# impromptuRong/hd_yolo

Hardware: AMD Instinct MI355X
Metric: tiles/sec (640x640) fwd+bwd (higher is better)
Workload: dtype bf16; 1 GPU; metayolo yolov5s 8-class nuclei, 640x640 RGB tiles, batch 64/GPU, train step = fwd + DetLoss + bwd + all-reduce + SGD(nesterov); global_batch=64, parallelism=dp1, world_size=1, backend=none, hw_queues=4

## Files before the change

### hd_yolo_amd/_ext.py

```python
import os

from . import _header, _lib
from ._header import HdyError

MEASURE_HEADER = os.path.join(os.path.dirname(_header.HEADER_PATH), 'hdyolo_measure.h')
_M = _header.read(MEASURE_HEADER)
SIGNATURES = _M.functions
PARAMS = _M.params
CONSTANTS = _M.constants
MEASURE_REVISION, MEASURE_COLS, MEASURE_MAX_SIDE = (CONSTANTS['HDY_MEASURE_' + n] for n in ('REVISION', 'COLS', 'MAX_SIDE'))

_bound = None


def load():
    global _bound
    lib = _lib.load()
    if _bound is not lib:
        rebuild = 'rebuild with `python -m hd_yolo_amd.build --force`'
        for name, (res, args) in SIGNATURES.items():
            fn = getattr(lib, name, None)
            if fn is None:
                raise HdyError(f'{_lib.LIB_PATH} does not export {name} (include/hdyolo_measure.h): it was built before the extension header '
                               f'existed; {rebuild}')
            fn.restype, fn.argtypes = res, args
        got = lib.hdy_measure_revision()
        if got != MEASURE_REVISION:
            raise HdyError(f'{_lib.LIB_PATH} was built for revision {got} of include/hdyolo_measure.h, this binding is written for '
                           f'{MEASURE_REVISION} (HDY_MEASURE_REVISION): {rebuild}')
        _bound = lib
    return lib


def call(name, *args):
    lib = load()
    rc = getattr(lib, name)(*args)
    if rc != 0:
        raise HdyError(f'{name} failed (status {rc}): {lib.hdy_last_error().decode()}')
```

### hd_yolo_amd/build.py

```python
import os
import subprocess
import sys
from concurrent.futures import ThreadPoolExecutor

HERE = os.path.dirname(os.path.abspath(__file__))
CSRC = os.path.join(HERE, 'csrc')
OUT = os.path.join(CSRC, 'build')
LIB = os.path.join(OUT, 'libhdyolo_hip.so')
SOURCES = ['api.hip', 'conv_dispatch.hip', 'conv_igemm.hip', 'conv3x3.hip', 'conv3x3_c128.hip', 'conv3x3s2.hip', 'conv_deep.hip', 'conv_stem.hip', 'conv_wgrad.hip', 'conv_wgrad3x3.hip', 'conv_wgrad_deep.hip', 'conv_dgrad_s2.hip', 'conv1x1_bwd.hip', 'bn_act.hip', 'pool.hip', 'detect.hip', 'nms_grid.hip', 'slide.hip', 'augment.hip', 'augment_masks.hip', 'score.hip', 'paste.hip', 'mask_score.hip', 'measure.hip', 'loss.hip', 'roi.hip', 'seg.hip', 'optim.hip', 'exec.hip']
FLAGS = ['--offload-arch=gfx950', '-O3', '-fPIC', '-std=c++17', '-ffp-contract=off', '-Wall', '-Wno-unused-function',
         '-I' + CSRC, '-I' + os.path.join(os.path.dirname(HERE), 'include')]


def _newer(a, bs):
    return os.path.exists(a) and all(os.path.getmtime(a) >= os.path.getmtime(b) for b in bs)


def build(force=False, verbose=True):
    os.makedirs(OUT, exist_ok=True)
    headers = [os.path.join(CSRC, h) for h in os.listdir(CSRC) if h.endswith('.h')]
    headers += [os.path.join(os.path.dirname(HERE), 'include', h) for h in ('hdyolo.h', 'hdyolo_measure.h')]
    hipcc = os.environ.get('HIPCC', '/opt/rocm/bin/hipcc')

    def compile_one(src):
        s = os.path.join(CSRC, src)
        o = os.path.join(OUT, src.replace('.hip', '.o'))
        if not force and _newer(o, [s] + headers):
            return o
        cmd = [hipcc] + FLAGS + ['-c', s, '-o', o]
        if verbose:
            print(' '.join(cmd), flush=True)
        subprocess.check_call(cmd)
        return o

    with ThreadPoolExecutor(max_workers=min(6, os.cpu_count() or 1)) as ex:
        objs = list(ex.map(compile_one, SOURCES))
    if force or not _newer(LIB, objs):
        cmd = [hipcc, '--offload-arch=gfx950', '-shared', '-fPIC', '-o', LIB] + objs
        if verbose:
            print(' '.join(cmd), flush=True)
        subprocess.check_call(cmd)
    return LIB


if __name__ == '__main__':
    print(build(force='--force' in sys.argv))
```

### hd_yolo_amd/csrc/api.hip

```cpp
#include <stdarg.h>
#include <stdio.h>
#include <stdlib.h>
#include <string.h>

#include <atomic>

#include "common.h"
#include "hdyolo_internal.h"
#include "hdyolo.h"

int hdy_pack_weight_launch(const hdy_pack_desc& d, hipStream_t st);
int hdy_pack_batch_launch(const hdy_pack_desc* table, int n, int total_blocks, hipStream_t st);

static thread_local char g_err[512] = "";

void hdy_set_error(const char* fmt, ...) {
    va_list ap;
    va_start(ap, fmt);
    vsnprintf(g_err, sizeof(g_err), fmt, ap);
    va_end(ap);
}

namespace {
struct OptDef { const char* name; int def; bool flag; };
const OptDef g_opt_def[HDY_OPT_COUNT] = {
    {"HDY_NO_CLASS_WALK", 0, true}, {"HDY_NO_CONV3X3", 0, true}, {"HDY_C3_GRID", 0, false}, {"HDY_NO_CONV3X3S2", 0, false},
    {"HDY_NO_DGRAD_S2", 0, false}, {"HDY_TILE_INTERLEAVE", 1, false}, {"HDY_NO_BIG_TILES", 0, true}, {"HDY_NO_STEM_KERNEL", 0, true},
    {"HDY_WGRAD_BLOCKS", 512, false}, {"HDY_NO_STEM_WGRAD", 0, true}, {"HDY_NO_WGRAD3X3", 0, true}, 
    {"HDY_LOSS_GRID", 2048, false}, {"HDY_NO_DEEP", 0, true}, {"HDY_NO_WGRAD_DEEP", 0, true}, {"HDY_DEEP_BN", 0, false}, {"HDY_DEEP_DEBUG", 0, false}, {"HDY_DEEP_ALL", 1, false}, {"HDY_DEEP_MIN_TILES", 160, false}, {"HDY_DEEP_WALK", 2, false}, {"HDY_NO_BN_REDUCE4", 0, true},
    {"HDY_WGRAD_TILE", 0, false}, {"HDY_SPPF_NO_KEYS", 0, true}, {"HDY_WGRAD_DEEP_KMIN", 192, false}, {"HDY_NO_CONV3X3_C128", 0, true}, {"HDY_NO_F1X1_96", 0, true},
    {"HDY_AP_CHUNK", 0, false}, {"HDY_AP_NO_PRUNE", 0, true},
};
std::atomic<int> g_opt[HDY_OPT_COUNT];
std::once_flag g_opt_once;
void opt_init() {
    std::call_once(g_opt_once, [] {
        for (int i = 0; i < HDY_OPT_COUNT; ++i) {
            const char* v = getenv(g_opt_def[i].name);
            g_opt[i].store(v ? (g_opt_def[i].flag ? 1 : atoi(v)) : g_opt_def[i].def, std::memory_order_relaxed);
        }
    });
}
int opt_index(const char* name) {
    for (int i = 0; name && i < HDY_OPT_COUNT; ++i)
        if (!strcmp(name, g_opt_def[i].name)) return i;
    return -1;
}
thread_local char g_disp_last[64] = "";
std::mutex g_disp_mu;
char g_disp_log[32768] = "";
size_t g_disp_len = 0;
thread_local char g_disp_copy[32768] = "";
}

int hdy_opt(int id) {
    opt_init();
    return g_opt[id].load(std::memory_order_relaxed);
}

void hdy_note_dispatch(const char* what) {
    snprintf(g_disp_last, sizeof(g_disp_last), "%s", what);
    const size_t n = strlen(g_disp_last);
    std::lock_guard<std::mutex> lock(g_disp_mu);
    if (g_disp_len + n + 2 < sizeof(g_disp_log)) {
// ... 148 lines not shown
```

### hd_yolo_amd/csrc/common.h

```cpp
#pragma once
#include <hip/hip_runtime.h>
#include <stdint.h>
#include <stddef.h>

#include <mutex>

#define HDY_OK 0
#define HDY_EINVAL (-1)
#define HDY_EUNSUPPORTED (-2)

enum { HDY_F32 = 0, HDY_BF16 = 1 };

void hdy_set_error(const char* fmt, ...);

enum HdyOption {
    HDY_OPT_NO_CLASS_WALK,
    HDY_OPT_NO_CONV3X3,
    HDY_OPT_C3_GRID,
    HDY_OPT_NO_CONV3X3S2,
    HDY_OPT_NO_DGRAD_S2,
    HDY_OPT_TILE_INTERLEAVE,
    HDY_OPT_NO_BIG_TILES,
    HDY_OPT_NO_STEM_KERNEL,
    HDY_OPT_WGRAD_BLOCKS,
    HDY_OPT_NO_STEM_WGRAD,
    HDY_OPT_NO_WGRAD3X3,
    HDY_OPT_LOSS_GRID,
    HDY_OPT_NO_DEEP,
    HDY_OPT_NO_WGRAD_DEEP,
    HDY_OPT_DEEP_BN,
    HDY_OPT_DEEP_DEBUG,
    HDY_OPT_DEEP_ALL,
    HDY_OPT_DEEP_MIN_TILES,
    HDY_OPT_DEEP_WALK,
    HDY_OPT_NO_BN_REDUCE4,
    HDY_OPT_WGRAD_TILE,
    HDY_OPT_SPPF_NO_KEYS,
    HDY_OPT_WGRAD_DEEP_KMIN,
    HDY_OPT_NO_CONV3X3_C128,
    HDY_OPT_NO_F1X1_96,
    HDY_OPT_AP_CHUNK,
    HDY_OPT_AP_NO_PRUNE,
    HDY_OPT_COUNT
};
int hdy_opt(int id);

void hdy_note_dispatch(const char* what);

#define HDY_ARG(cond, ...)                 \
    do {                                   \
        if (!(cond)) {                     \
            hdy_set_error(__VA_ARGS__);    \
            return HDY_EINVAL;             \
        }                                  \
    } while (0)

#define HDY_LAUNCH_CHECK(what)                                                       \
    do {                                                                             \
        hipError_t e__ = hipGetLastError();                                          \
        if (e__ != hipSuccess) {                                                     \
            hdy_set_error("%s: launch failed: %s", what, hipGetErrorString(e__));    \
            return (int)e__;                                                         \
        }                                                                            \
    } while (0)

typedef __bf16 bf16_t;
typedef int i32x4 __attribute__((ext_vector_type(4)));
typedef float f32x4 __attribute__((ext_vector_type(4)));
typedef __bf16 bf16x8 __attribute__((ext_vector_type(8)));
typedef __bf16 bf16x4 __attribute__((ext_vector_type(4)));

#if defined(__HIPCC__)
__device__ __forceinline__ float row_sum16(float v) {
#ifdef HDY_ROW_SUM_SHFL
    for (int m = 1; m < 16; m <<= 1) v += __shfl_xor(v, m);
// ... 131 lines not shown
```

### hd_yolo_amd/csrc/exec.hip

```cpp
#include <hip/hip_runtime.h>
#include <stdlib.h>
#include <string.h>

#include <mutex>
#include <tuple>
#include <type_traits>
#include <utility>
#include <vector>

#include "common.h"
#include "hdyolo.h"

namespace {

typedef unsigned long long u64;

#define HDY_HIP(call)                                                                  \
    do {                                                                               \
        hipError_t e__ = (call);                                                       \
        if (e__ != hipSuccess) {                                                       \
            hdy_set_error("exec: %s failed: %s", #call, hipGetErrorString(e__));       \
            return (int)e__;                                                           \
        }                                                                              \
    } while (0)

template <typename T>
T arg_from(u64 v) {
    if constexpr (std::is_pointer_v<T>) {
        return reinterpret_cast<T>((uintptr_t)v);
    } else if constexpr (std::is_same_v<T, float>) {
        const unsigned u = (unsigned)v;
        float f;
        __builtin_memcpy(&f, &u, 4);
        return f;
    } else if constexpr (std::is_same_v<T, double>) {
        double d;
        __builtin_memcpy(&d, &v, 8);
        return d;
    } else {
        static_assert(std::is_integral_v<T>, "entry point parameter that is neither pointer, integer nor floating point");
        return static_cast<T>(v);
    }
}

template <typename... P, size_t... I>
int call_impl(int (*f)(P...), const u64* a, void* stream, std::index_sequence<I...>) {
    using Tup = std::tuple<P...>;
    return f(arg_from<std::tuple_element_t<I, Tup>>(a[I])..., stream);
}

template <typename... P>
int invoke(int (*f)(P...), const u64* a, int nargs, void* stream) {
    static_assert(sizeof...(P) >= 1, "no stream parameter");
    static_assert(std::is_same_v<std::tuple_element_t<sizeof...(P) - 1, std::tuple<P...>>, void*>, "the last parameter must be the stream");
    if (nargs != (int)sizeof...(P) - 1) return -1000 - (int)sizeof...(P);
    return call_impl(f, a, stream, std::make_index_sequence<sizeof...(P) - 1>{});
}

struct Entry {
    const char* name;
    int (*run)(const u64*, int, void*);
};
#define E(fn) {#fn, [](const u64* a, int n, void* s) { return invoke(&fn, a, n, s); }}
const Entry TABLE[] = {
    E(hdy_conv_pack), E(hdy_conv_pack_run), E(hdy_conv_fwd), E(hdy_conv_dgrad), E(hdy_conv_wgrad), E(hdy_conv_dgrad_stats),
    E(hdy_conv1x1_bwd_fused_stats), E(hdy_bn_bwd_finalize_slabs), E(hdy_bn_act_bwd_apply), E(hdy_conv1x1_bwd_fused), E(hdy_bn_finalize),
    E(hdy_bn_eval_coeffs), E(hdy_bn_eval_coeffs_batch), E(hdy_bn_act_fwd), E(hdy_bn_act_bwd), E(hdy_bn_finalize_pair), E(hdy_bn_act_fwd_pair),
    E(hdy_bn_act_bwd_pair), E(hdy_add_inplace), E(hdy_colsum), E(hdy_sppf_pool_fwd), E(hdy_sppf_pool_bwd), E(hdy_upsample2x_fwd),
    E(hdy_upsample2x_bwd), E(hdy_stem_prep), E(hdy_nchw_to_nhwc), E(hdy_decode), E(hdy_det_grad_pack), E(hdy_nms_batched), E(hdy_det_outputs),
    E(hdy_nms_boxes), E(hdy_roi_align_fwd), E(hdy_roi_align_bwd), E(hdy_relu_bwd), E(hdy_cast_store), E(hdy_det_loss), E(hdy_mask_select),
    E(hdy_det_targets), E(hdy_scale_inplace), E(hdy_groupnorm_fwd), E(hdy_groupnorm_bwd), E(hdy_bilinear_fwd), E(hdy_bilinear_bwd),
    E(hdy_bilinear_bwd_axis), E(hdy_softdice), E(hdy_softdice_wgrad), E(hdy_softmax2d), E(hdy_conv_wgrad_stem_fused), E(hdy_bn_slab_sums),
    E(hdy_bn_finalize_sums), E(hdy_bn_bwd_coeffs_sums), E(hdy_copy_f32), E(hdy_det_loss_ex),
    E(hdy_nms_grid_begin), E(hdy_nms_grid_round), E(hdy_nms_grid_finish), E(hdy_slide_tiles_u8), E(hdy_slide_append), E(hdy_slide_tissue_u8),
    E(hdy_augment_tiles_u8), E(hdy_augment_boxes), E(hdy_augment_mask_extents), E(hdy_augment_boxes_masks), E(hdy_augment_mask_targets),
    E(hdy_ap_match), E(hdy_paste_masks), E(hdy_paste_label_map), E(hdy_label_areas),
    E(hdy_label_overlap), E(hdy_mask_ap_match), E(hdy_roi_align_levels_fwd), E(hdy_mask_rows), E(hdy_opt_step),
};
#undef E
constexpr int NTABLE = (int)(sizeof(TABLE) / sizeof(TABLE[0]));

struct TokenEvents {
    hipEvent_t start = nullptr, done = nullptr;
};
std::mutex g_ev_mutex;
std::vector<std::vector<TokenEvents>> g_events;

int events_for(u64 token, TokenEvents* out) {
    if (token >= 65536) return HDY_EINVAL;
    int dev = 0;
    if (hipGetDevice(&dev) != hipSuccess) return HDY_EINVAL;
    std::lock_guard<std::mutex> lock(g_ev_mutex);
    if ((int)g_events.size() <= dev) g_events.resize(dev + 1);
    auto& v = g_events[dev];
    if (v.size() <= token) v.resize(token + 1);
    TokenEvents& t = v[token];
    if (!t.start) {
        static const unsigned flags = hipEventDisableTiming | (getenv("HDY_EVENT_SYSTEM_SCOPE") ? 0u : (unsigned)hipEventReleaseToDevice);
        if (hipEventCreateWithFlags(&t.start, flags) != hipSuccess || hipEventCreateWithFlags(&t.done, flags) != hipSuccess) return HDY_EINVAL;
    }
    *out = t;
    return HDY_OK;
}

int run_words(const u64* w, size_t n, hipStream_t main, hipStream_t side, hipStream_t on, bool in_fork) {
    size_t i = 0;
    while (i < n) {
        HDY_ARG(i + 2 <= n, "exec: truncated item at word %zu", i);
        const u64 op = w[i], nargs = w[i + 1];
        HDY_ARG(nargs <= 64 && i + 2 + nargs <= n, "exec: item at word %zu has %llu arguments, %zu words left", i, nargs, n - i - 2);
// ... 65 lines not shown
```

### hd_yolo_amd/ops.py

```python
import ctypes
import struct
import os
import threading

import torch

from . import _lib
from ._lib import ACT_NONE, ACT_RELU, ACT_SILU, BF16, F32, PACK_DGRAD, PACK_FWD, PACK_STEM

BN_EPS, BN_MOMENTUM = 1e-3, 0.03


def _rec(scope, name, args):
    return (name, args, tuple(v for v in scope.values() if isinstance(v, torch.Tensor)) +
            tuple(t for v in scope.values() if isinstance(v, (list, tuple)) for t in v if isinstance(t, torch.Tensor)))


def dcode(dtype):
    if dtype == torch.float32:
        return F32
    if dtype == torch.bfloat16:
        return BF16
    raise _lib.HdyError(f'unsupported arithmetic type {dtype}: use torch.float32 or torch.bfloat16')


def stat_slabs(N, H, W, C, K, R, S, stride, pad, dtype):
    return _lib.query('hdy_conv_stat_slabs', N, H, W, C, K, R, S, stride, pad, dcode(dtype))


def require_gpu(t):
    if not t.is_cuda:
        raise _lib.HdyError('hd_yolo_amd runs on MI355X only: tensor is on CPU and there is no CPU fallback '
                            '(the CPU oracle under oracle/ is test infrastructure)')


def nhwc(t):
    require_gpu(t)
    assert t.dim() == 4 and (t.shape[3] == 1 or t.stride(3) == 1), f'not NHWC-contiguous in C: {t.shape} {t.stride()}'
    n, h, w, c = t.shape
    ld = t.stride(2)
# ... 79 lines not shown
            base = cls._next_token
            cls._next_token += n
            return base

    def __del__(self):
        n = getattr(self, '_ntok', 0)
        if n:
            with Program._lock:
                fr = sorted(Program._free + [(self.token_base, n)])
                merged = []
                for base, cnt in fr:
                    if merged and merged[-1][0] + merged[-1][1] == base:
                        merged[-1] = (merged[-1][0], merged[-1][1] + cnt)
                    else:
                        merged.append((base, cnt))
                if merged and merged[-1][0] + merged[-1][1] == Program._next_token:
                    Program._next_token = merged.pop()[0]
                Program._free[:] = merged

    def __init__(self, records):
        lib = _lib.load()
        self.records = records
        self.nrec = len(records)
        self.side = None
        self.segments = []
        words = []
        ntok = 1 + max([r[3] for r in records if r[0] == '@fork'] + [r[2] for r in records if r[0] == '@join'] + [0])
        self.token_base = Program._take_tokens(ntok)
        self._ntok = ntok

        def item(rec):
            name, args = rec[0], rec[1]
            op = lib.hdy_exec_op(name.encode())
            types = _lib.SIGNATURES[name][1]
            if op < 0 or len(args) != len(types) - 1:
                raise _lib.HdyError(f'{name} cannot be listed for hdy_exec_run ({len(args)} arguments recorded, {len(types) - 1} expected: '
                                    f'{", ".join(p for p, _ in _lib.PARAMS[name][:-1])})')
            return [op, len(args)] + [_word(v, t) for v, t in zip(args, types)]

        def flush():
            if words:
                self.segments.append(('words', (ctypes.c_ulonglong * len(words))(*words), len(words)))
                del words[:]

        for rec in records:
            name = rec[0]
            if name == '@call':
                flush()
                self.segments.append(('call', rec[1]))
            elif name in ('@fork', '@join'):
                if self.side is not None and self.side is not rec[1]:
                    raise _lib.HdyError('a launch list forks onto one side stream')
                self.side = rec[1]
                if name == '@join':
                    words.extend([EXEC_JOIN, 1, self.token_base + rec[2]])
                else:
                    body = [w for r in rec[2] for w in item(r)]
                    words.extend([EXEC_FORK, 2, self.token_base + rec[3], len(body)] + body)
            else:
                words.extend(item(rec))
        flush()

    def run(self):
        lib = _lib.load()
        main = stream_ptr()
        side = self.side.stream.cuda_stream if self.side is not None else None
        for seg in self.segments:
            if seg[0] == 'call':
                seg[1]()
                continue
# ... 62 lines not shown
def out_dim(n, k, s, p):
    return (n + 2 * p - k) // s + 1


def pack_alloc(K, C, R, S, stride, pad, kind, dtype, device):
    n = _lib.query('hdy_conv_pack_elems', K, C, R, S, stride, pad, kind, dcode(dtype))
    return torch.empty(n, dtype=dtype, device=device)


def rec_pack(w_a, w_b, stride, pad, kind, out, K=None):
    K_a, C, R, S = w_a.shape
    K_b = 0 if w_b is None else w_b.shape[0]
    K = K_a + K_b if K is None else K
    assert w_a.is_contiguous() and w_a.dtype == torch.float32 and (w_b is None or (w_b.is_contiguous() and w_b.shape[1:] == w_a.shape[1:]))
    return _rec(locals(), 'hdy_conv_pack', (ptr(w_a), K_a, ptr(w_b), K_b, K, C, R, S, stride, pad, kind, dcode(out.dtype), ptr(out)))


def rec_conv_fwd(x, wp, y, K, R, S, stride, pad, scale=None, shift=None, stats=None, act=ACT_NONE, accumulate=False,
                 stem_hw=None, res=None):
    xp, N, H, W, C, ldx = nhwc(x)
    yp, _, Ho, Wo, Ky, ldy = nhwc(y)
    stem = 0
    if stem_hw is not None:
        stem, (H, W), C = 1, stem_hw, 3
    assert Ky == K and Ho == out_dim(H, R, stride, pad) and Wo == out_dim(W, S, stride, pad), (y.shape, K, Ho, Wo)
    out_f32 = 1 if (y.dtype == torch.float32 and x.dtype == torch.bfloat16) else 0
    assert y.dtype == x.dtype or out_f32
    rp, ldr = None, 0
    if res is not None:
        rp, _, _, _, Kr, ldr = nhwc(res)
        assert Kr == K and res.dtype == y.dtype and res.shape == y.shape
    return _rec(locals(), 'hdy_conv_fwd', (xp, ldx, ptr(wp), ptr(scale), ptr(shift), rp, ldr, yp, ldy, ptr(stats), 0 if stats is None else stats.shape[0], N, H, W, C, K, R, S, stride, pad, act,
                             int(accumulate), dcode(x.dtype), out_f32, stem))


class StatRequest:

    def __init__(self, y, scale, shift, slabs, c0, act):
        yp, _, _, _, K, ldy = nhwc(y)
        for t in (scale, shift):
            assert t.dtype == torch.float32 and t.numel() >= K and t.stride(0) == 1
        assert slabs.dtype == torch.float32 and slabs.is_contiguous() and slabs.shape[1:] == (2, K)
        self.c = _lib.StatReq(yp, ldy, ptr(scale), ptr(shift), ptr(slabs), c0, c0 + K, act, slabs.shape[0])
        self.keep = (y, scale, shift, slabs)


def _stat_array(stats):
    arr = (_lib.StatReq * len(stats))(*[q.c for q in stats])
    return arr, ctypes.cast(arr, ctypes.c_void_p)


def conv_dgrad_stat_slabs(N, H, W, C, K, R, S, stride, pad, dtype):
    return _lib.query('hdy_conv_dgrad_stat_slabs', N, H, W, C, K, R, S, stride, pad, dcode(dtype))


def rec_conv_dgrad(dy, wp_d, dx, R, S, stride, pad, accumulate=False, stats=None):
    dyp, N, Ho, Wo, K, lddy = nhwc(dy)
    dxp, _, H, W, C, lddx = nhwc(dx)
    assert Ho == out_dim(H, R, stride, pad) and Wo == out_dim(W, S, stride, pad) and dy.dtype == dx.dtype
    if stats:
        arr, arrp = _stat_array(stats)
        keep = [t for q in stats for t in q.keep]
        return _rec(locals(), 'hdy_conv_dgrad_stats', (dyp, lddy, ptr(wp_d), dxp, lddx, N, H, W, C, K, R, S, stride, pad, int(accumulate), dcode(dy.dtype),
                                                       arrp, len(stats))) + ((arr,),)
    return _rec(locals(), 'hdy_conv_dgrad', (dyp, lddy, ptr(wp_d), dxp, lddx, N, H, W, C, K, R, S, stride, pad, int(accumulate), dcode(dy.dtype)))

# ... 1141 lines not shown
```

### hd_yolo_amd/plan.py

```python
import os

import torch
import torch.nn as nn

from . import _lib, ops

USE_GRAPHS = os.environ.get('HDY_GRAPH', '0') == '1'
SIDE_WGRAD = os.environ.get('HDY_SIDE_WGRAD', '1') == '1' and not USE_GRAPHS
DY_RING = int(os.environ.get('HDY_DY_RING', '4'))
SKIP_WGRAD = os.environ.get('HDY_SKIP_WGRAD') == '1'
PRODUCER_STATS = os.environ.get('HDY_PRODUCER_STATS', 'fused')
STEM_FUSED = os.environ.get('HDY_STEM_FUSED', '1') == '1'
FUSED_1X1 = os.environ.get('HDY_FUSED_1X1', '1') == '1'
PACK_SIDE = os.environ.get('HDY_PACK_SIDE', '0') == '1'
FORK_MIN_PIXELS = int(os.environ.get('HDY_FORK_MIN_PIXELS', '0'))
GRAD_BUCKET_BYTES = int(os.environ.get('HDY_GRAD_BUCKET_MB', '6')) << 20


class Val:
    __slots__ = ('n', 'h', 'w', 'c', 'name', 'buf', 'off', 'cat', 'parts', 'gbuf', 'goff', 'ginit', 'galias', 'gfinal',
                 'order', 'last_use', 'index', 'needs_grad')

    def __init__(self, n, h, w, c, name, order):
        self.n, self.h, self.w, self.c, self.name, self.order = n, h, w, c, name, order
# ... 121 lines not shown

def act_code(act):
    if isinstance(act, nn.SiLU):
        return ops.ACT_SILU
    if isinstance(act, nn.Identity):
        return ops.ACT_NONE
    raise _lib.HdyError(f'activation {type(act).__name__} has no HIP kernel on this path (SiLU / Identity only)')


def _is(m, name):
    return type(m).__name__ == name


class Plan:
    def __init__(self, backbone, neck, head, shape, dtype, training, device, grad_store=None, taps=(), tap_params=(), sync=None):
        self.dtype, self.training, self.device = dtype, training, device
        self.sync = sync if training else None
        self.ext_shapes = dict(shape) if isinstance(shape, dict) else None
        if self.ext_shapes is not None:
            if backbone is not None or training:
                raise _lib.HdyError('feature-input plans are neck/head-only and forward-only')
            self.B, self.Cin, self.H, self.W = next(iter(self.ext_shapes.values()))[0], 0, 0, 0
        else:
            self.B, self.Cin, self.H, self.W = shape
        self.input = None
        self.ext = {}
        self.vals, self.units = [], []
        self.grad_store = grad_store
        self.tap_keys, self.tap_params = list(taps), list(tap_params)
        self.tap_grads_ready = False
        self.bucket_hook = None
        self._order = 0
        self._trace(backbone, neck, head)
        self._allocate()
        self.packs = ops.PackTable(device)
        self.bn_eval = ops.BnEvalTable(device)
        self.fwd = self._compile_forward()
        self.bwd = self._compile_backward() if training else None
        self._graphs = {'fwd': None, 'bwd': None}
        self._runs = {'fwd': 0, 'bwd': 0}
        self._progs = {}
        self._bn_running = None
        self._pack_stream = None

    def _val(self, n, h, w, c, name):
        v = Val(n, h, w, c, name, self._order)
        self._order += 1
        self.vals.append(v)
        return v

    def _use(self, v):
        v.last_use = self._order

    def _conv(self, mods, x, res=None, stem=False):
        c0 = mods[0].conv
        for m in mods:
            c = m.conv
            if c.groups != 1 or c.dilation[0] != 1 or c.kernel_size[0] != c.kernel_size[1] or c.stride[0] != c.stride[1]:
                raise _lib.HdyError('grouped / dilated / non-square convolutions are outside the hot path')
            assert (c.kernel_size, c.stride, c.padding, c.in_channels) == (c0.kernel_size, c0.stride, c0.padding, c0.in_channels)
        k, s, p = c0.kernel_size[0], c0.stride[0], c0.padding[0]
        if stem:
            n, h, w = self.B, self.H, self.W
        else:
            n, h, w = x.n, x.h, x.w
            self._use(x)
# ... 104 lines not shown
                cur.index = m.i
                outs[m.i] = cur
            self.feature_keys = list(neck.save)
        self.outs = outs
        heads = [] if head is None else (list(head) if isinstance(head, (list, tuple)) else [head])
        self.det_units, self.det_split = [], []
        for hi, hd in enumerate(heads):
            f = hd.f if isinstance(hd.f, (list, tuple)) else [hd.f]
            for l, (j, conv) in enumerate(zip(f, hd.m)):
                self._use(outs[j])
                u = DetUnit(conv, outs[j], l)
                u.head, u.na, u.no = hi, hd.na, hd.no
                self.units.append(u)
                self.det_units.append(u)
            self.det_split.append(len(f))
        if heads:
            self.na, self.no = heads[0].na, heads[0].no
        if len(heads) > 1 and any(getattr(hd, 'seg', None) is not None for hd in heads):
            raise _lib.HdyError('a mask branch is supported on single-header models only')
        head = heads[0] if len(heads) == 1 else None
        self.mask_vals = []
        if head is not None and getattr(head, 'seg', None) is not None:
            f = head.f if isinstance(head.f, (list, tuple)) else [head.f]
            vals = [self._module(m, outs[f[-i]]) for i, m in enumerate(head.seg, 1)]
            self.mask_vals = vals[::-1]
        self.mask_grads_ready = False
        self.seg_h_params = list(head.seg_h.parameters()) if self.mask_vals else []

    def _fusable_1x1(self, u):
        return (FUSED_1X1 and not USE_GRAPHS and self.training and self.dtype == torch.bfloat16 and not u.stem and u.k == 1 and u.s == 1
                and u.p == 0 and u.has_bn and not u.frozen and u.act == ops.ACT_SILU and ops.fused_1x1_ok(u.C, u.K, self.dtype)
                and all(m.conv.out_channels % 8 == 0 for m in u.mods))

    def _new(self, *shape, dtype=None, zero=False):
        f = torch.zeros if zero else torch.empty
        return f(shape, dtype=dtype or self.dtype, device=self.device)

    def _allocate(self):
        self._alloc_activations()
        need = _Scratch()
        alloc = {ConvUnit: self._alloc_conv, DetUnit: self._alloc_det, PoolUnit: self._alloc_pool}
        for u in self.units:
            if type(u) in alloc:
                alloc[type(u)](u, need)
        if self.training:
            self._alloc_det_grads()
            self._alloc_scratch(need)
            self._alloc_gradients()

    def _alloc_activations(self):
        for v in self.vals:
            if v.parts is not None or v.cat is None:
                v.buf = self._new(v.n, v.h, v.w, v.c)
        for v in self.vals:
            if v.cat is not None:
                v.buf = v.cat.buf
        self.prep = self._new(self.B, self.H + 4, self.W + 4, 4)

    def _alloc_conv(self, u, need):
        dt, f32, o = self.dtype, torch.float32, u.outs[0]
        u.wp = ops.pack_alloc(u.K, u.C, u.k, u.k, u.s, u.p, u.pack_kind, dt, self.device)
        u.scale, u.shift = self._new(u.K, dtype=f32), self._new(u.K, dtype=f32)
        if not self.training:
            return
        if not u.has_bn:
            raise _lib.HdyError('training a fused (BN-folded) model is not supported: build the model unfused')
        u.yraw = self._new(o.n, o.h, o.w, u.K)
        if u.frozen:
            u.mean = u.invstd = None
            u.mtiles = 0
        else:
            u.mean, u.invstd = self._new(u.K, dtype=f32), self._new(u.K, dtype=f32)
            u.mtiles = ops.stat_slabs(o.n, u.hin, u.win, u.C, u.K, u.k, u.k, u.s, u.p, dt)
        need.add(stats=u.mtiles * 2 * u.K, dy=u.M * u.K, bnws=ops.bn_bwd_ws_floats(u.M, u.K), kmax=u.K,
                 wg=ops.wgrad_ws_bytes(o.n, u.hin, u.win, u.C, u.K, u.k, u.k, u.s, u.p, dt, stem=u.stem))
        if self._fusable_1x1(u):
            need.add(f1=ops.fused_1x1_ws_bytes(u.M, u.C, u.K))
        if not u.stem:
            u.wpd = ops.pack_alloc(u.K, u.C, u.k, u.k, u.s, u.p, ops.PACK_DGRAD, dt, self.device)

    def _alloc_det(self, u, need):
        x, dt = u.x, self.dtype
        u.wp = ops.pack_alloc(u.K, x.c, 1, 1, 1, 0, ops.PACK_FWD, dt, self.device)
        u.logits = self._new(x.n, x.h, x.w, u.Kp, dtype=torch.float32, zero=True)
        if self.training:
            u.wpd = ops.pack_alloc(u.Kp, x.c, 1, 1, 1, 0, ops.PACK_DGRAD, dt, self.device)
            need.add(wg=ops.wgrad_ws_bytes(x.n, x.h, x.w, x.c, u.Kp, 1, 1, 1, 0, dt), bnws=ops.bn_bwd_ws_floats(u.M, u.Kp))

    def _alloc_pool(self, u, need):
        if self.training:
            a = u.x
            u.idx = [self._new(a.n, a.h, a.w, a.c, dtype=torch.uint8) for _ in range(3)]

    def _alloc_det_grads(self):
        sizes = [u.M * u.Kp for u in self.det_units]
        self.gdet_flat = self._new(max(sum(sizes), 1), zero=True)
        off = 0
        for u, n in zip(self.det_units, sizes):
            u.gdet = self.gdet_flat[off:off + n].view(u.x.n, u.x.h, u.x.w, u.Kp)
            off += n
        self.loss_out = self._new(4, dtype=torch.float32, zero=True)
        self.loss_call = None

    def _alloc_scratch(self, need):
        f32 = torch.float32
        self.stats = self._new(need.stats, dtype=f32)
# ... 32 lines not shown
        recs = []
        for u in self.units:
            emit[type(u)](recs, u)
        return recs

    def _fwd_pool(self, recs, u):
        recs.append(ops.rec_sppf_pool_fwd(u.x.t(), u.outs[0].t(), u.outs[1].t(), u.outs[2].t(), u.idx if self.training else None))

    def _fwd_up(self, recs, u):
        recs.append(ops.rec_upsample_fwd(u.x.t(), u.out.t()))

    def _fwd_det(self, recs, u):
        self.packs.add(u.conv.weight, None, 1, 0, ops.PACK_FWD, u.wp)
        recs.append(ops.rec_conv_fwd(u.x.t(), u.wp, u.logits[..., :u.K], u.K, 1, 1, 1, 0, shift=u.conv.bias))

    def _fwd_conv(self, recs, u):
        (self._fwd_conv_train if self.training else self._fwd_conv_eval)(recs, u, self.prep if u.stem else u.x.t())

    def _fwd_conv_eval(self, recs, u, x):
        m, o = u.mods[0], u.outs[0]
        self.packs.add(m.conv.weight, None, u.s, u.p, u.pack_kind, u.wp)
        if u.has_bn:
            self.bn_eval.add(*self._bn(m), u.scale, u.shift, eps=m.bn.eps)
            scale, shift = u.scale, u.shift
        else:
            scale, shift = None, m.conv.bias
        res = u.res.t() if u.res is not None else None
        recs.append(ops.rec_conv_fwd(x, u.wp, o.t(), u.K, u.k, u.k, u.s, u.p, scale=scale, shift=shift, act=u.act, stem_hw=u.stem_hw, res=res))

    def _fwd_conv_train(self, recs, u, x):
        wb = u.mods[1].conv.weight if len(u.mods) > 1 else None
        self.packs.add(u.mods[0].conv.weight, wb, u.s, u.p, u.pack_kind, u.wp)
        stats = None if u.frozen else self.stats[:u.mtiles * 2 * u.K].view(u.mtiles, 2, u.K)
        recs.append(ops.rec_conv_fwd(x, u.wp, u.yraw, u.K, u.k, u.k, u.s, u.p, stats=stats, stem_hw=u.stem_hw))
        getattr(self, '_bn_fwd_' + self._bn_fwd_mode(u))(recs, u, stats)

    def _bn_fwd_mode(self, u):
        if self.sync and not u.frozen:
            return 'sync'
        if self._pair_apply(u):
            return 'pair'
        return 'frozen' if u.frozen else 'single'

    @staticmethod
    def _pair_apply(u):
        return len(u.mods) == 2 and not u.frozen and u.res is None

    def _bn_fwd_apply(self, recs, u, coeffs=None):
        pair = self._pair_apply(u)
        res = u.res.t() if u.res is not None else None
        for m, o, ch in self._channels(u):
            if coeffs is not None:
                recs.append(coeffs(m, ch.start, ch.stop - ch.start))
            if not pair:
                recs.append(ops.rec_bn_act_fwd(u.yraw[..., ch], u.scale[ch], u.shift[ch], o.t(), res=res, act=u.act))
        if pair:
            recs.append(ops.rec_bn_act_fwd_pair(u.yraw, u.scale, u.shift, u.outs[0].t(), u.outs[1].t(), act=u.act))

    def _bn_fwd_sync(self, recs, u, stats):
        buf = self.sync_sums[:2 * u.K + 1]
        recs.append(ops.rec_bn_slab_sums(stats, u.mtiles, u.K, u.M, buf))
        recs.append(self._sync_call(buf))
        self._bn_fwd_apply(recs, u, lambda m, k0, K: ops.rec_bn_finalize_sums(
            buf, u.K, k0, K, K, self._bn(m), None, u.scale[k0:], u.shift[k0:], u.mean[k0:], u.invstd[k0:], eps=m.bn.eps, momentum=m.bn.momentum))

    def _bn_fwd_pair(self, recs, u, stats):
        ma, mb = u.mods
        assert ma.bn.eps == mb.bn.eps and ma.bn.momentum == mb.bn.momentum
        recs.append(ops.rec_bn_finalize_pair(stats, u.mtiles, u.K, ma.conv.out_channels, u.M, self._bn(ma), self._bn(mb), u.scale, u.shift,
                                             u.mean, u.invstd, eps=ma.bn.eps, momentum=ma.bn.momentum, ws=self.fin_ws))
        self._bn_fwd_apply(recs, u)

    def _bn_fwd_single(self, recs, u, stats):
        self._bn_fwd_apply(recs, u, lambda m, k0, K: ops.rec_bn_finalize(
            stats[:, :, k0:], u.mtiles, K, u.M, *self._bn(m), u.scale[k0:], u.shift[k0:], u.mean[k0:], u.invstd[k0:], stats_ld=u.K, ws=self.fin_ws))

    def _bn_fwd_frozen(self, recs, u, stats):
        self._bn_fwd_apply(recs, u, lambda m, k0, K: ops.rec_bn_eval_coeffs(*self._bn(m), u.scale[k0:k0 + K], u.shift[k0:k0 + K], eps=m.bn.eps))

    def _replay(self, key, recs):
        if not USE_GRAPHS:
            if not ops.USE_EXEC:
                return ops.run(recs)
            prog = self._progs.get(key)
            if prog is None or prog.records is not recs or prog.nrec != len(recs):
                prog = self._progs[key] = ops.Program(recs)
            return prog.run()
# ... 377 lines not shown
```

Before: 5561 tiles/s.

## Add dedicated 1x1 conv forward kernel with fused BN-on-load of producer

Adds a specialised bf16 MFMA kernel for stride-1 1x1 convolutions with C,K in {32,64,128} and at least a minimum row count in training. It keeps the filter in registers, double-buffers row loads and writes per-block BN statistic slabs. Where the producer conv has a single reader and a plain BN, the kernel applies the producer's BN+activation on load, also writes the activated tensor, and skips the separate bn_act_fwd pass. The aim is to cut launches and memory round trips, at the cost of more dispatch complexity and a new plan path for graph aliasing.

Result: no change. 5611 tiles/s (median of 6 runs) (+0.9%).

```diff
diff --git a/hd_yolo_amd/_ext.py b/hd_yolo_amd/_ext.py
--- a/hd_yolo_amd/_ext.py
+++ b/hd_yolo_amd/_ext.py
@@ -10,6 +10,13 @@
 CONSTANTS = _M.constants
 MEASURE_REVISION, MEASURE_COLS, MEASURE_MAX_SIDE = (CONSTANTS['HDY_MEASURE_' + n] for n in ('REVISION', 'COLS', 'MAX_SIDE'))
 
+CONV1X1_HEADER = os.path.join(os.path.dirname(_header.HEADER_PATH), 'hdyolo_conv1x1.h')
+_C = _header.read(CONV1X1_HEADER)
+CONV1X1_SIGNATURES, CONV1X1_PARAMS = _C.functions, _C.params
+CONV1X1_REVISION = _C.constants['HDY_CONV1X1_REVISION']
+_EXTENSIONS = (('hdyolo_measure.h', SIGNATURES, MEASURE_REVISION, 'hdy_measure_revision'),
+               ('hdyolo_conv1x1.h', CONV1X1_SIGNATURES, CONV1X1_REVISION, 'hdy_conv1x1_revision'))
+
 _bound = None
 
 
@@ -18,16 +25,16 @@
     lib = _lib.load()
     if _bound is not lib:
         rebuild = 'rebuild with `python -m hd_yolo_amd.build --force`'
-        for name, (res, args) in SIGNATURES.items():
-            fn = getattr(lib, name, None)
-            if fn is None:
-                raise HdyError(f'{_lib.LIB_PATH} does not export {name} (include/hdyolo_measure.h): it was built before the extension header '
-                               f'existed; {rebuild}')
-            fn.restype, fn.argtypes = res, args
-        got = lib.hdy_measure_revision()
-        if got != MEASURE_REVISION:
-            raise HdyError(f'{_lib.LIB_PATH} was built for revision {got} of include/hdyolo_measure.h, this binding is written for '
-                           f'{MEASURE_REVISION} (HDY_MEASURE_REVISION): {rebuild}')
+        for header, sigs, revision, getter in _EXTENSIONS:
+            for name, (res, args) in sigs.items():
+                fn = getattr(lib, name, None)
+                if fn is None:
+                    raise HdyError(f'{_lib.LIB_PATH} does not export {name} (include/{header}): it was built before the extension header '
+                                   f'existed; {rebuild}')
+                fn.restype, fn.argtypes = res, args
+            got = getattr(lib, getter)()
+            if got != revision:
+                raise HdyError(f'{_lib.LIB_PATH} was built for revision {got} of include/{header}, this binding is written for {revision}: {rebuild}')
         _bound = lib
     return lib
 
diff --git a/hd_yolo_amd/build.py b/hd_yolo_amd/build.py
--- a/hd_yolo_amd/build.py
+++ b/hd_yolo_amd/build.py
@@ -7,7 +7,7 @@
 CSRC = os.path.join(HERE, 'csrc')
 OUT = os.path.join(CSRC, 'build')
 LIB = os.path.join(OUT, 'libhdyolo_hip.so')
-SOURCES = ['api.hip', 'conv_dispatch.hip', 'conv_igemm.hip', 'conv3x3.hip', 'conv3x3_c128.hip', 'conv3x3s2.hip', 'conv_deep.hip', 'conv_stem.hip', 'conv_wgrad.hip', 'conv_wgrad3x3.hip', 'conv_wgrad_deep.hip', 'conv_dgrad_s2.hip', 'conv1x1_bwd.hip', 'bn_act.hip', 'pool.hip', 'detect.hip', 'nms_grid.hip', 'slide.hip', 'augment.hip', 'augment_masks.hip', 'score.hip', 'paste.hip', 'mask_score.hip', 'measure.hip', 'loss.hip', 'roi.hip', 'seg.hip', 'optim.hip', 'exec.hip']
+SOURCES = ['api.hip', 'conv_dispatch.hip', 'conv_igemm.hip', 'conv3x3.hip', 'conv3x3_c128.hip', 'conv3x3s2.hip', 'conv_deep.hip', 'conv_stem.hip', 'conv_wgrad.hip', 'conv_wgrad3x3.hip', 'conv_wgrad_deep.hip', 'conv_dgrad_s2.hip', 'conv1x1_bwd.hip', 'conv1x1_fwd.hip', 'bn_act.hip', 'pool.hip', 'detect.hip', 'nms_grid.hip', 'slide.hip', 'augment.hip', 'augment_masks.hip', 'score.hip', 'paste.hip', 'mask_score.hip', 'measure.hip', 'loss.hip', 'roi.hip', 'seg.hip', 'optim.hip', 'exec.hip']
 FLAGS = ['--offload-arch=gfx950', '-O3', '-fPIC', '-std=c++17', '-ffp-contract=off', '-Wall', '-Wno-unused-function',
          '-I' + CSRC, '-I' + os.path.join(os.path.dirname(HERE), 'include')]
 
@@ -19,7 +19,7 @@
 def build(force=False, verbose=True):
     os.makedirs(OUT, exist_ok=True)
     headers = [os.path.join(CSRC, h) for h in os.listdir(CSRC) if h.endswith('.h')]
-    headers += [os.path.join(os.path.dirname(HERE), 'include', h) for h in ('hdyolo.h', 'hdyolo_measure.h')]
+    headers += [os.path.join(os.path.dirname(HERE), 'include', h) for h in ('hdyolo.h', 'hdyolo_measure.h', 'hdyolo_conv1x1.h')]
     hipcc = os.environ.get('HIPCC', '/opt/rocm/bin/hipcc')
 
     def compile_one(src):
diff --git a/hd_yolo_amd/csrc/api.hip b/hd_yolo_amd/csrc/api.hip
--- a/hd_yolo_amd/csrc/api.hip
+++ b/hd_yolo_amd/csrc/api.hip
@@ -29,7 +29,7 @@
     {"HDY_WGRAD_BLOCKS", 512, false}, {"HDY_NO_STEM_WGRAD", 0, true}, {"HDY_NO_WGRAD3X3", 0, true}, 
     {"HDY_LOSS_GRID", 2048, false}, {"HDY_NO_DEEP", 0, true}, {"HDY_NO_WGRAD_DEEP", 0, true}, {"HDY_DEEP_BN", 0, false}, {"HDY_DEEP_DEBUG", 0, false}, {"HDY_DEEP_ALL", 1, false}, {"HDY_DEEP_MIN_TILES", 160, false}, {"HDY_DEEP_WALK", 2, false}, {"HDY_NO_BN_REDUCE4", 0, true},
     {"HDY_WGRAD_TILE", 0, false}, {"HDY_SPPF_NO_KEYS", 0, true}, {"HDY_WGRAD_DEEP_KMIN", 192, false}, {"HDY_NO_CONV3X3_C128", 0, true}, {"HDY_NO_F1X1_96", 0, true},
-    {"HDY_AP_CHUNK", 0, false}, {"HDY_AP_NO_PRUNE", 0, true},
+    {"HDY_AP_CHUNK", 0, false}, {"HDY_AP_NO_PRUNE", 0, true}, {"HDY_NO_CONV1X1_FWD", 0, false}, {"HDY_CONV1X1_FWD_MIN_ROWS", 32768, false},
 };
 std::atomic<int> g_opt[HDY_OPT_COUNT];
 std::once_flag g_opt_once;
diff --git a/hd_yolo_amd/csrc/common.h b/hd_yolo_amd/csrc/common.h
--- a/hd_yolo_amd/csrc/common.h
+++ b/hd_yolo_amd/csrc/common.h
@@ -41,6 +41,8 @@
     HDY_OPT_NO_F1X1_96,
     HDY_OPT_AP_CHUNK,
     HDY_OPT_AP_NO_PRUNE,
+    HDY_OPT_NO_CONV1X1_FWD,
+    HDY_OPT_CONV1X1_FWD_MIN_ROWS,
     HDY_OPT_COUNT
 };
 int hdy_opt(int id);
diff --git a/hd_yolo_amd/csrc/conv1x1_fwd.hip b/hd_yolo_amd/csrc/conv1x1_fwd.hip
--- /dev/null
+++ b/hd_yolo_amd/csrc/conv1x1_fwd.hip
@@ -0,0 +1,277 @@
+#include <type_traits>
+
+#include "common.h"
+#include "hdyolo.h"
+#include "hdyolo_conv1x1.h"
+
+namespace {
+
+__device__ __forceinline__ float fast_silu(float u) { return u * fast_sigmoid(u); }
+
+struct F1Args {
+    const bf16_t* x; int ldx;
+    const float *scale, *shift;
+    bf16_t* z; int ldz;
+    const bf16_t* w; int Kdp;
+    bf16_t* y; int ldy;
+    int M;
+    float* stats;
+};
+
+template <int C, int K, bool BN> struct Cfg {
+    static constexpr int NS = (C == 128 && K == 128) ? 2 : 1;
+    static constexpr int KS = C / 32, KW = K / NS, KF = KW / 16;
+    static constexpr bool BIG = C * K > 64 * 64 || K == 128;
+    static constexpr int MINWG = BIG ? 2 : 3;
+    static constexpr int U = C == 128 ? (BN ? 1 : NS) : (BN ? 64 : 128) / C;
+    static constexpr bool LDS_COEF = BN && C == 128;
+};
+
+template <int C, int K, bool BN, int ACT>
+__global__ __launch_bounds__(256, (Cfg<C, K, BN>::MINWG)) void conv1x1_fwd_kernel(const F1Args p) {
+    typedef Cfg<C, K, BN> G;
+    constexpr int KS = G::KS, KF = G::KF, U = G::U, NS = G::NS, KW = G::KW;
+    __shared__ __attribute__((aligned(16))) float sRed[16 * 2 * K];
+    __shared__ __attribute__((aligned(16))) float sCoef[G::LDS_COEF ? 2 * C : 4];
+
+    const int tid = threadIdx.x, lane = tid & 63, wave = tid >> 6;
+    const int fr = lane & 15, fq = lane >> 4;
+    const int gw = (blockIdx.x * 4 + wave) / NS, GW = gridDim.x * 4 / NS;
+    const int cb = (wave % NS) * KW;
+    const int tiles = (p.M + 15) >> 4;
+    const int nt = gw < tiles ? (tiles - gw + GW - 1) / GW : 0;
+
+    V16 bw[KF][KS];
+#pragma unroll
+    for (int j = 0; j < KF; ++j)
+#pragma unroll
+        for (int ks = 0; ks < KS; ++ks) bw[j][ks].i = *(const i32x4*)(p.w + (size_t)(cb + fr * KF + j) * p.Kdp + (ks * 4 + fq) * 8);
+
+    float sc[G::LDS_COEF ? 1 : KS][8], sh[G::LDS_COEF ? 1 : KS][8];
+    if constexpr (BN) {
+        if constexpr (G::LDS_COEF) {
+            if (tid < C) sCoef[tid] = p.scale[tid];
+            else if (tid < 2 * C) sCoef[tid] = p.shift[tid - C];
+            __syncthreads();
+        } else {
+#pragma unroll
+            for (int ks = 0; ks < KS; ++ks)
+#pragma unroll
+                for (int i = 0; i < 8; ++i) {
+                    sc[ks][i] = p.scale[(ks * 4 + fq) * 8 + i];
+                    sh[ks][i] = p.shift[(ks * 4 + fq) * 8 + i];
+                }
+        }
+    }
+
+    const unsigned coef_lds = (unsigned)(uintptr_t)(const __attribute__((address_space(3))) float*)sCoef + fq * 32;
+    (void)coef_lds;
+
+    float s1[KF], s2[KF];
+#pragma unroll
+    for (int j = 0; j < KF; ++j) { s1[j] = 0.f; s2[j] = 0.f; }
+
+    auto issue = [&](i32x4* slot, int i) {
+        const int m = min((i * GW + gw) * 16 + fr, p.M - 1);
+        const bf16_t* src = p.x + (size_t)m * p.ldx + fq * 8;
+#pragma unroll
+        for (int ks = 0; ks < KS; ++ks) slot[ks] = *(const i32x4*)(src + ks * 32);
+    };
+    auto process = [&](auto guard, const i32x4* slot, int i) {
+        constexpr bool GUARD = decltype(guard)::value;
+        __builtin_amdgcn_sched_barrier(0);
+        const int m0 = (i * GW + gw) * 16;
+        const bool ok_in = !GUARD || m0 + fr < p.M;
+        V16 a[KS];
+#pragma unroll
+        for (int ks = 0; ks < KS; ++ks) {
+            a[ks].i = slot[ks];
+            if constexpr (BN) {
+                if constexpr (G::BIG) __builtin_amdgcn_sched_barrier(0);
+                float v[8], cs[8], ch[8];
+                if constexpr (G::LDS_COEF) {
+                    f32x4 c0, c1, h0, h1;
+                    asm volatile("ds_read_b128 %0, %1 offset:%2" : "=v"(c0) : "v"(coef_lds), "n"(ks * 128));
+                    asm volatile("ds_read_b128 %0, %1 offset:%2" : "=v"(c1) : "v"(coef_lds), "n"(ks * 128 + 16));
+                    asm volatile("ds_read_b128 %0, %1 offset:%2" : "=v"(h0) : "v"(coef_lds), "n"(C * 4 + ks * 128));
+                    asm volatile("ds_read_b128 %0, %1 offset:%2" : "=v"(h1) : "v"(coef_lds), "n"(C * 4 + ks * 128 + 16));
+                    asm volatile("s_waitcnt lgkmcnt(0)" : "+v"(c0), "+v"(c1), "+v"(h0), "+v"(h1));
+#pragma unroll
+                    for (int e = 0; e < 4; ++e) { cs[e] = c0[e]; cs[4 + e] = c1[e]; ch[e] = h0[e]; ch[4 + e] = h1[e]; }
+                } else {
+#pragma unroll
+                    for (int e = 0; e < 8; ++e) { cs[e] = sc[ks][e]; ch[e] = sh[ks][e]; }
+                }
+                unpack<bf16_t>(a[ks].i, v);
+#pragma unroll
+                for (int e = 0; e < 8; ++e) {
+                    float u = v[e] * cs[e] + ch[e];
+                    if (ACT == 1) u = fast_silu(u);
+                    else if (ACT == 2) u = u < 0.0f ? 0.0f : u;
+                    v[e] = u;
+                }
+                a[ks].i = pack<bf16_t>(v);
+                if (ok_in && (NS == 1 || cb == 0)) *(i32x4*)(p.z + (size_t)(m0 + fr) * p.ldz + (ks * 4 + fq) * 8) = a[ks].i;
+            }
+            if (GUARD && !ok_in) a[ks].i = i32x4{0, 0, 0, 0};
+        }
+        constexpr int JG = KF < 4 ? 2 : 4;
+#pragma unroll
+        for (int j0 = 0; j0 < KF; j0 += JG) {
+            __builtin_amdgcn_sched_barrier(0);
+            f32x4 acc[JG];
+#pragma unroll
+            for (int j = 0; j < JG; ++j) {
+                acc[j] = f32x4{0.f, 0.f, 0.f, 0.f};
+#pragma unroll
+                for (int ks = 0; ks < KS; ++ks) acc[j] = __builtin_amdgcn_mfma_f32_16x16x32_bf16(a[ks].h, bw[j0 + j][ks].h, acc[j], 0, 0, 0);
+            }
+#pragma unroll
+            for (int j = 0; j < JG; ++j)
+#pragma unroll
+                for (int r = 0; r < 4; ++r) {
+                    const float v = acc[j][r];
+                    s1[j0 + j] += v;
+                    s2[j0 + j] = __builtin_fmaf(v, v, s2[j0 + j]);
+                }
+#pragma unroll
+            for (int r = 0; r < 4; ++r) {
+                const int m = m0 + fq * 4 + r;
+                if (!GUARD || m < p.M) {
+                    bf16_t* dst = p.y + (size_t)m * p.ldy + cb + fr * KF + j0;
+                    if constexpr (JG == 4) {
+                        const bf16x4 o = {(bf16_t)acc[0][r], (bf16_t)acc[1][r], (bf16_t)acc[2][r], (bf16_t)acc[3][r]};
+                        *(bf16x4*)dst = o;
+                    } else {
+                        typedef __bf16 bf16x2 __attribute__((ext_vector_type(2)));
+                        const bf16x2 o = {(bf16_t)acc[0][r], (bf16_t)acc[1][r]};
+                        *(bf16x2*)dst = o;
+                    }
+                }
+            }
+        }
+    };
+
+    const int ragged = (p.M & 15) != 0 && nt > 0 && (nt - 1) * GW + gw == tiles - 1;
+    const int ntf = nt - ragged;
+    auto issue_set = [&](i32x4 (*set)[KS], int i) {
+#pragma unroll
+        for (int u = 0; u < U; ++u) issue(set[u], i + u);
+    };
+    auto process_set = [&](i32x4 (*set)[KS], int i) {
+#pragma unroll
+        for (int u = 0; u < U; ++u) process(std::false_type{}, set[u], i + u);
+    };
+    i32x4 setA[U][KS], setB[U][KS];
+    int i = 0;
+    if (U <= ntf) issue_set(setA, 0);
+    for (; i + 3 * U <= ntf; i += 2 * U) {
+        issue_set(setB, i + U);
+        process_set(setA, i);
+        issue_set(setA, i + 2 * U);
+        process_set(setB, i + U);
+    }
+    if (i + U <= ntf) {
+        const bool two = i + 2 * U <= ntf;
+        if (two) issue_set(setB, i + U);
+        process_set(setA, i);
+        i += U;
+        if (two) {
+            process_set(setB, i);
+            i += U;
+        }
+    }
+    const int rem = nt - i;
+#pragma unroll
+    for (int u = 0; u < U; ++u)
+        if (u < rem) issue(setA[u], i + u);
+#pragma unroll
+    for (int u = 0; u < U; ++u)
+        if (u < rem) process(std::true_type{}, setA[u], i + u);
+
+    if (p.stats) {
+        float* mine = sRed + (wave * 4 + fq) * 2 * K + cb + fr * KF;
+#pragma unroll
+        for (int j = 0; j < KF; ++j) {
+            mine[j] = s1[j];
+            mine[K + j] = s2[j];
+        }
+        __syncthreads();
+        for (int o = tid; o < 2 * K; o += 256) {
+            const int h = (o % K) / KW;
+            float s = 0.f;
+#pragma unroll
+            for (int q = 0; q < 16 / NS; ++q) s += sRed[(((q >> 2) * NS + h) * 4 + (q & 3)) * 2 * K + o];
+            p.stats[(size_t)blockIdx.x * 2 * K + o] = s;
+        }
+    }
+}
+
+template <int C, int K, bool BN, int ACT>
+void launch_ck(const F1Args& a, int grid, hipStream_t st) {
+    hipLaunchKernelGGL((conv1x1_fwd_kernel<C, K, BN, ACT>), dim3(grid), dim3(256), 0, st, a);
+}
+template <int C, int K>
+void launch_mode(const F1Args& a, int act, int grid, hipStream_t st) {
+    if (!a.scale) launch_ck<C, K, false, 0>(a, grid, st);
+    else if (act == HDY_ACT_SILU) launch_ck<C, K, true, 1>(a, grid, st);
+    else if (act == HDY_ACT_RELU) launch_ck<C, K, true, 2>(a, grid, st);
+    else launch_ck<C, K, true, 0>(a, grid, st);
+}
+template <int C>
+void launch_c(const F1Args& a, int K, int act, int grid, hipStream_t st) {
+    if (K == 32) launch_mode<C, 32>(a, act, grid, st);
+    else if (K == 64) launch_mode<C, 64>(a, act, grid, st);
+    else launch_mode<C, 128>(a, act, grid, st);
+}
+
+inline bool width_ok(int n) { return n == 32 || n == 64 || n == 128; }
+
+int grid_of(long long M, int C, int K) {
+    const long long tiles = (M + 15) / 16;
+    const int ns = C == 128 && K == 128 ? 2 : 1;
+    const long long cap = 256 * (C * K > 64 * 64 || K == 128 ? 2 : 3) * 4 / ns;
+    const long long per = (tiles + cap - 1) / cap;
+    return (int)(((tiles + per - 1) / per * ns + 3) / 4);
+}
+
+}
+
+extern "C" {
+
+int hdy_conv1x1_revision(void) { return HDY_CONV1X1_REVISION; }
+
+int hdy_conv1x1_fwd_stat_slabs(long long M, int C, int K) {
+    if (hdy_opt(HDY_OPT_NO_CONV1X1_FWD) == 1 || !width_ok(C) || !width_ok(K) || M <= 0 || M >= (1LL << 31) - 16) return 0;
+    return grid_of(M, C, K);
+}
+
+int hdy_conv1x1_fwd(const void* x, int ldx, const float* scale, const float* shift, int act, void* z, int ldz, const void* w_packed, void* y,
+                    int ldy, long long M, int C, int K, float* stats, int nslabs, int dtype, void* stream) {
+    if (hdy_opt(HDY_OPT_NO_CONV1X1_FWD) == 1 || dtype != HDY_BF16 || !width_ok(C) || !width_ok(K)) {
+        hdy_set_error("conv1x1_fwd: declined (bf16, C and K in {32, 64, 128}, HDY_NO_CONV1X1_FWD != 1): C=%d K=%d dtype=%d", C, K, dtype);
+        return HDY_EUNSUPPORTED;
+    }
+    HDY_ARG(x && w_packed && y && M > 0 && M < (1LL << 31) - 16, "conv1x1_fwd: bad args");
+    HDY_ARG(ldx >= C && ldx % 8 == 0 && ldy >= K && ldy % 8 == 0, "conv1x1_fwd: pitches must be >= the width and multiples of 8 elements (ldx=%d ldy=%d)", ldx, ldy);
+    HDY_ARG((((uintptr_t)x | (uintptr_t)y | (uintptr_t)w_packed) & 15) == 0, "conv1x1_fwd: x, y and the packed filter must be 16-byte aligned");
+    const bool bn = scale || shift || z;
+    HDY_ARG(!bn || (scale && shift && z), "conv1x1_fwd: BatchNorm on load needs scale, shift and z");
+    HDY_ARG(!bn || (ldz >= C && ldz % 8 == 0 && ((uintptr_t)z & 15) == 0 && act >= HDY_ACT_NONE && act <= HDY_ACT_RELU), "conv1x1_fwd: bad z / act (ldz=%d act=%d)", ldz, act);
+    HDY_ARG(bn || act == HDY_ACT_NONE, "conv1x1_fwd: an activation needs BatchNorm on load");
+    const int grid = grid_of(M, C, K);
+    HDY_ARG((stats == nullptr && nslabs == 0) || (stats && nslabs == grid), "conv1x1_fwd: the statistics array holds %d slabs, this launch writes %d", nslabs, grid);
+    F1Args a;
+    a.x = (const bf16_t*)x; a.ldx = ldx; a.scale = scale; a.shift = shift; a.z = (bf16_t*)z; a.ldz = ldz;
+    a.w = (const bf16_t*)w_packed; a.Kdp = round_up(C, 64);
+    a.y = (bf16_t*)y; a.ldy = ldy; a.M = (int)M; a.stats = stats;
+    static const char* const names[2][3] = {{"conv1x1_fwd_c32", "conv1x1_fwd_c64", "conv1x1_fwd_c128"}, {"conv1x1_fwd_c32_bn", "conv1x1_fwd_c64_bn", "conv1x1_fwd_c128_bn"}};
+    hdy_note_dispatch(names[bn][C == 32 ? 0 : (C == 64 ? 1 : 2)]);
+    if (C == 32) launch_c<32>(a, K, act, grid, (hipStream_t)stream);
+    else if (C == 64) launch_c<64>(a, K, act, grid, (hipStream_t)stream);
+    else launch_c<128>(a, K, act, grid, (hipStream_t)stream);
+    HDY_LAUNCH_CHECK("conv1x1_fwd");
+    return HDY_OK;
+}
+
+}
diff --git a/hd_yolo_amd/csrc/exec.hip b/hd_yolo_amd/csrc/exec.hip
--- a/hd_yolo_amd/csrc/exec.hip
+++ b/hd_yolo_amd/csrc/exec.hip
@@ -10,6 +10,7 @@
 
 #include "common.h"
 #include "hdyolo.h"
+#include "hdyolo_conv1x1.h"
 
 namespace {
 
@@ -75,7 +76,7 @@
     E(hdy_nms_grid_begin), E(hdy_nms_grid_round), E(hdy_nms_grid_finish), E(hdy_slide_tiles_u8), E(hdy_slide_append), E(hdy_slide_tissue_u8),
     E(hdy_augment_tiles_u8), E(hdy_augment_boxes), E(hdy_augment_mask_extents), E(hdy_augment_boxes_masks), E(hdy_augment_mask_targets),
     E(hdy_ap_match), E(hdy_paste_masks), E(hdy_paste_label_map), E(hdy_label_areas),
-    E(hdy_label_overlap), E(hdy_mask_ap_match), E(hdy_roi_align_levels_fwd), E(hdy_mask_rows), E(hdy_opt_step),
+    E(hdy_label_overlap), E(hdy_mask_ap_match), E(hdy_roi_align_levels_fwd), E(hdy_mask_rows), E(hdy_opt_step), E(hdy_conv1x1_fwd),
 };
 #undef E
 constexpr int NTABLE = (int)(sizeof(TABLE) / sizeof(TABLE[0]));
diff --git a/hd_yolo_amd/ops.py b/hd_yolo_amd/ops.py
--- a/hd_yolo_amd/ops.py
+++ b/hd_yolo_amd/ops.py
@@ -5,7 +5,7 @@
 
 import torch
 
-from . import _lib
+from . import _ext, _lib
 from ._lib import ACT_NONE, ACT_RELU, ACT_SILU, BF16, F32, PACK_DGRAD, PACK_FWD, PACK_STEM
 
 BN_EPS, BN_MOMENTUM = 1e-3, 0.03
@@ -151,10 +151,11 @@
         def item(rec):
             name, args = rec[0], rec[1]
             op = lib.hdy_exec_op(name.encode())
-            types = _lib.SIGNATURES[name][1]
+            ext = name not in _lib.SIGNATURES
+            types = (_ext.CONV1X1_SIGNATURES if ext else _lib.SIGNATURES)[name][1]
             if op < 0 or len(args) != len(types) - 1:
                 raise _lib.HdyError(f'{name} cannot be listed for hdy_exec_run ({len(args)} arguments recorded, {len(types) - 1} expected: '
-                                    f'{", ".join(p for p, _ in _lib.PARAMS[name][:-1])})')
+                                    f'{", ".join(p for p, _ in (_ext.CONV1X1_PARAMS if ext else _lib.PARAMS)[name][:-1])})')
             return [op, len(args)] + [_word(v, t) for v, t in zip(args, types)]
 
         def flush():
@@ -283,6 +284,24 @@
         assert Kr == K and res.dtype == y.dtype and res.shape == y.shape
     return _rec(locals(), 'hdy_conv_fwd', (xp, ldx, ptr(wp), ptr(scale), ptr(shift), rp, ldr, yp, ldy, ptr(stats), 0 if stats is None else stats.shape[0], N, H, W, C, K, R, S, stride, pad, act,
                              int(accumulate), dcode(x.dtype), out_f32, stem))
+
+
+def conv1x1_fwd_stat_slabs(M, C, K):
+    return _ext.load().hdy_conv1x1_fwd_stat_slabs(M, C, K)
+
+
+def rec_conv1x1_fwd(x, wp, y, stats=None, scale=None, shift=None, act=ACT_NONE, z=None):
+    xp, N, H, W, C, ldx = nhwc(x)
+    yp, _, _, _, K, ldy = nhwc(y)
+    assert y.shape[:3] == x.shape[:3] and y.dtype == x.dtype
+    zp, ldz = None, 0
+    if z is not None:
+        zp, _, _, _, Cz, ldz = nhwc(z)
+        assert Cz == C and z.shape[:3] == x.shape[:3] and z.dtype == x.dtype and scale is not None and shift is not None
+    assert stats is None or (stats.dtype == torch.float32 and stats.is_contiguous() and tuple(stats.shape[1:]) == (2, K))
+    _ext.load()
+    return _rec(locals(), 'hdy_conv1x1_fwd', (xp, ldx, ptr(scale), ptr(shift), act, zp, ldz, ptr(wp), yp, ldy, N * H * W, C, K, ptr(stats),
+                                              0 if stats is None else stats.shape[0], dcode(x.dtype)))
 
 
 class StatRequest:
diff --git a/hd_yolo_amd/plan.py b/hd_yolo_amd/plan.py
--- a/hd_yolo_amd/plan.py
+++ b/hd_yolo_amd/plan.py
@@ -177,6 +177,7 @@
         self.bucket_hook = None
         self._order = 0
         self._trace(backbone, neck, head)
+        self._select_conv1x1_fwd()
         self._allocate()
         self.packs = ops.PackTable(device)
         self.bn_eval = ops.BnEvalTable(device)
@@ -347,6 +348,30 @@
                 and u.p == 0 and u.has_bn and not u.frozen and u.act == ops.ACT_SILU and ops.fused_1x1_ok(u.C, u.K, self.dtype)
                 and all(m.conv.out_channels % 8 == 0 for m in u.mods))
 
+    def _select_conv1x1_fwd(self):
+        opt = _lib.query('hdy_get_option', b'HDY_NO_CONV1X1_FWD')
+        min_rows = _lib.query('hdy_get_option', b'HDY_CONV1X1_FWD_MIN_ROWS')
+        convs = [u for u in self.units if isinstance(u, ConvUnit)]
+        for u in convs:
+            u.bn_src = u.bn_by = None
+            u.f1fwd = (opt != 1 and self.training and self.dtype == torch.bfloat16 and not u.stem and u.k == 1 and u.s == 1 and u.p == 0
+                       and u.has_bn and u.C in (32, 64, 128) and u.K in (32, 64, 128) and u.M >= min_rows)
+        readers, producer = {}, {}
+        for u in self.units:
+            ins = [u.x] + ([u.res] if isinstance(u, ConvUnit) and u.res is not None else [])
+            for v in ins:
+                if v is not None:
+                    readers[id(v)] = readers.get(id(v), 0) + 1
+            if isinstance(u, ConvUnit):
+                for o in u.outs:
+                    producer[id(o)] = u
+        outside = {id(self.outs[k]) for k in list(self.tap_keys) + list(self.feature_keys) if k in self.outs} | {id(v) for v in self.mask_vals}
+        for u in convs:
+            x, q = u.x, producer.get(id(u.x))
+            if (u.f1fwd and (u.C <= 64 or opt == 2) and q is not None and len(q.mods) == 1 and self._bn_fwd_mode(q) == 'single' and q.res is None
+                    and readers.get(id(x)) == 1 and x.cat is None and x.parts is None and x.galias is None and id(x) not in outside):
+                u.bn_src, q.bn_by = q, u
+
     def _new(self, *shape, dtype=None, zero=False):
         f = torch.zeros if zero else torch.empty
         return f(shape, dtype=dtype or self.dtype, device=self.device)
@@ -386,7 +411,8 @@
             u.mtiles = 0
         else:
             u.mean, u.invstd = self._new(u.K, dtype=f32), self._new(u.K, dtype=f32)
-            u.mtiles = ops.stat_slabs(o.n, u.hin, u.win, u.C, u.K, u.k, u.k, u.s, u.p, dt)
+            u.mtiles = (ops.conv1x1_fwd_stat_slabs(u.M, u.C, u.K) if u.f1fwd else
+                        ops.stat_slabs(o.n, u.hin, u.win, u.C, u.K, u.k, u.k, u.s, u.p, dt))
         need.add(stats=u.mtiles * 2 * u.K, dy=u.M * u.K, bnws=ops.bn_bwd_ws_floats(u.M, u.K), kmax=u.K,
                  wg=ops.wgrad_ws_bytes(o.n, u.hin, u.win, u.C, u.K, u.k, u.k, u.s, u.p, dt, stem=u.stem))
         if self._fusable_1x1(u):
@@ -485,7 +511,12 @@
         wb = u.mods[1].conv.weight if len(u.mods) > 1 else None
         self.packs.add(u.mods[0].conv.weight, wb, u.s, u.p, u.pack_kind, u.wp)
         stats = None if u.frozen else self.stats[:u.mtiles * 2 * u.K].view(u.mtiles, 2, u.K)
-        recs.append(ops.rec_conv_fwd(x, u.wp, u.yraw, u.K, u.k, u.k, u.s, u.p, stats=stats, stem_hw=u.stem_hw))
+        if u.f1fwd:
+            q = u.bn_src
+            on_load = {} if q is None else dict(scale=q.scale, shift=q.shift, act=q.act, z=x)
+            recs.append(ops.rec_conv1x1_fwd(x if q is None else q.yraw, u.wp, u.yraw, stats=stats, **on_load))
+        else:
+            recs.append(ops.rec_conv_fwd(x, u.wp, u.yraw, u.K, u.k, u.k, u.s, u.p, stats=stats, stem_hw=u.stem_hw))
         getattr(self, '_bn_fwd_' + self._bn_fwd_mode(u))(recs, u, stats)
 
     def _bn_fwd_mode(self, u):
@@ -505,7 +536,7 @@
         for m, o, ch in self._channels(u):
             if coeffs is not None:
                 recs.append(coeffs(m, ch.start, ch.stop - ch.start))
-            if not pair:
+            if not pair and u.bn_by is None:
                 recs.append(ops.rec_bn_act_fwd(u.yraw[..., ch], u.scale[ch], u.shift[ch], o.t(), res=res, act=u.act))
         if pair:
             recs.append(ops.rec_bn_act_fwd_pair(u.yraw, u.scale, u.shift, u.outs[0].t(), u.outs[1].t(), act=u.act))
diff --git a/include/hdyolo_conv1x1.h b/include/hdyolo_conv1x1.h
--- /dev/null
+++ b/include/hdyolo_conv1x1.h
@@ -0,0 +1,20 @@
+#ifndef HDYOLO_CONV1X1_H
+#define HDYOLO_CONV1X1_H
+
+#include <stddef.h>
+#include <stdint.h>
+
+#ifdef __cplusplus
+extern "C" {
+#endif
+
+#define HDY_CONV1X1_REVISION 1
+int hdy_conv1x1_revision(void);
+int hdy_conv1x1_fwd_stat_slabs(long long M, int C, int K);
+int hdy_conv1x1_fwd(const void* x, int ldx, const float* scale, const float* shift, int act, void* z, int ldz, const void* w_packed, void* y,
+                    int ldy, long long M, int C, int K, float* stats, int nslabs, int dtype, void* stream);
+
+#ifdef __cplusplus
+}
+#endif
+#endif
```
